# Yukun-Huang/DreamWaltz-G

Hardware: AMD Instinct MI355X
Metric: SDS steps/sec @512^2, 100k Gaussians, SD1.5+ControlNet; raster Mpix/s vs HBM roofline (higher is better)
Workload: dtype f32x

## Files before the change

dreamwaltz-g_amd/csrc/gemm.hip:

```cpp
#include "dwg_common.h"
#include "dwg_prof_internal.h"
#include "../../include/dwg_gemm.h"
#include <cstdlib>
#include <type_traits>

#if defined(DWG_GEMM_X_TU)
#include "dwg_xfmt.h"
typedef _Float16 HT;
#define DWG_DTYPE_HALF DWG_DTYPE_F32X
#define DWG_MFMA16(a, b, c) __builtin_amdgcn_mfma_f32_32x32x16_f16(a, b, c, 0, 0, 0)
#define DWG_HALF_NAME "f32x"
#elif defined(DWG_GEMM_F16_TU)
typedef _Float16 HT;
#define DWG_DTYPE_HALF DWG_DTYPE_F16
#define DWG_MFMA16(a, b, c) __builtin_amdgcn_mfma_f32_32x32x16_f16(a, b, c, 0, 0, 0)
#define DWG_HALF_NAME "f16"
#else
typedef __bf16 HT;
#define DWG_DTYPE_HALF DWG_DTYPE_BF16
#define DWG_MFMA16(a, b, c) __builtin_amdgcn_mfma_f32_32x32x16_bf16(a, b, c, 0, 0, 0)
#define DWG_HALF_NAME "bf16"
#endif

namespace {

typedef __attribute__((ext_vector_type(8))) HT bf16x8;
typedef __attribute__((ext_vector_type(16))) float f32x16;

struct ConvP {
    int enabled, Cin, Hin, Win, Hout, Wout, KH, KW, stride, pad_t, pad_l, dil;
    int up;
    int cin1;
    const void* A2;
};

struct GemmP {
    const void* A; const void* B; void* C; const void* bias; const void* residual;
    int M, N, K;
    long long sam, sak, sbn, sbk, ldc, ldr;
    int nb2;
    long long bA1, bA2, bB1, bB2, bC1, bC2, bR1, bR2;
    int act; float alpha;
    int out_bf16, res_bf16, bias_per_row, splitk, accumulate;
    float* ws;
    int bias_row_div;
    long long bias_ld;
    ConvP conv;
};

__device__ __forceinline__ float bf2f(HT x) { return (float)x; }
__device__ __forceinline__ HT f2bf(float x) { return (HT)x; }

struct bf16x4_t { HT v[4]; };
#ifdef DWG_GEMM_X_TU
__device__ __forceinline__ float ld_half1(const void* base, long long i) { return dwg_x_get1(base, i); }
__device__ __forceinline__ void st_half1(void* base, long long i, float v) { dwg_x_put1(base, i, v); }
__device__ __forceinline__ void ld_half4(const void* base, long long i, float (&v)[4]) { dwg_x_get4(base, i, v); }
__device__ __forceinline__ void st_half4(void* base, long long i, const float (&v)[4]) { dwg_x_put4(base, i, v); }
#else
__device__ __forceinline__ float ld_half1(const void* base, long long i) { return bf2f(reinterpret_cast<const HT*>(base)[i]); }
__device__ __forceinline__ void st_half1(void* base, long long i, float v) { reinterpret_cast<HT*>(base)[i] = f2bf(v); }
__device__ __forceinline__ void ld_half4(const void* base, long long i, float (&v)[4]) {
    const bf16x4_t r = *reinterpret_cast<const bf16x4_t*>(reinterpret_cast<const HT*>(base) + i);
// ... 59 lines not shown

    __device__ __forceinline__ void init(const T* base_, long long srow_, long long sk_, int nrows_, int r0_, int kbeg, int kend_,
                                         const ConvP& cv) {
        base = base_; srow = srow_; sk = sk_; nrows = nrows_; r0 = r0_; kend = kend_;
        const int tid = threadIdx.x;
        if (MODE == MODE_KVEC) {
            kcur = kbeg + (tid % CPR) * VEC;
#pragma unroll
            for (int i = 0; i < NCH; i++) {
                int r = r0 + tid / CPR + i * RPI;
                rowptr[i] = r < nrows ? base + (long long)r * srow : nullptr;
            }
        } else if (MODE == MODE_CONV) {
            kcur = kbeg + (tid % CPR) * VEC;
            const int hw = cv.Hout * cv.Wout;
#pragma unroll
            for (int i = 0; i < NCH; i++) {
                int r = r0 + tid / CPR + i * RPI;
                rok[i] = r < nrows;
                int rr = rok[i] ? r : 0;
                int img = rr / hw, rem = rr - img * hw;
                int oy = rem / cv.Wout, ox = rem - oy * cv.Wout;
                iy0[i] = oy * cv.stride - cv.pad_t; ix0[i] = ox * cv.stride - cv.pad_l;
                pix0[i] = (long long)img * cv.Hin * cv.Win;
            }
            int tap = kcur / cv.Cin;
            ci = kcur - tap * cv.Cin; ky = tap / cv.KW; kx = tap - ky * cv.KW;
        } else {
            kcur = kbeg;
        }
    }

    __device__ __forceinline__ void advance(const ConvP& cv) {
        kcur += BK;
        if (MODE == MODE_CONV) {
            ci += BK;
            while (ci >= cv.Cin) { ci -= cv.Cin; if (++kx == cv.KW) { kx = 0; ++ky; } }
        }
// ... 75 lines not shown
        acc = DWG_MFMA16(a, b, acc);
    }
}
template <>
__device__ __forceinline__ void mma_tile<float>(const float* sa, const float* sb, int lane, f32x16& acc) {
    constexpr int LDT = TT<float>::BK + TT<float>::PAD;
    const float* pa = sa + (lane & 31) * LDT + (lane >> 5);
    const float* pb = sb + (lane & 31) * LDT + (lane >> 5);
#pragma unroll
    for (int ks = 0; ks < TT<float>::BK / 2; ks++)
        acc = __builtin_amdgcn_mfma_f32_32x32x2f32(pa[ks * 2], pb[ks * 2], acc, 0, 0, 0);
}

template <bool LIGHT = false>
__device__ __forceinline__ void epilogue_store(const GemmP& p, float v, int row, int col, long long coff, long long roff) {
    const long long ci = coff + (long long)row * p.ldc + col;
    if (p.bias) v += reinterpret_cast<const float*>(p.bias)[p.bias_row_div > 0 ? (long long)(row / p.bias_row_div) * p.bias_ld + col
                                                                             : (p.bias_per_row ? row : col)];
    v = apply_act<LIGHT>(v, p.act);
    if (p.residual) {
        const long long ri = roff + (long long)row * p.ldr + col;
        v += p.res_bf16 ? ld_half1(p.residual, ri) : reinterpret_cast<const float*>(p.residual)[ri];
    }
    if (p.out_bf16) st_half1(p.C, ci, v);
    else if (p.accumulate) reinterpret_cast<float*>(p.C)[ci] += v;
    else reinterpret_cast<float*>(p.C)[ci] = v;
}

__device__ __forceinline__ bool epilogue_vec_ok(const GemmP& p, long long coff, long long roff) {
    bool ok = (p.N & 3) == 0 && (p.ldc & 3) == 0 && (coff & 3) == 0 && ((uintptr_t)p.C & 15) == 0;
    if (p.residual) ok = ok && (p.ldr & 3) == 0 && (roff & 3) == 0 && ((uintptr_t)p.residual & 15) == 0;
    return ok;
}

template <bool LIGHT = false>
__device__ __forceinline__ void epilogue_store4(const GemmP& p, float (&v)[4], int row, int col, long long coff, long long roff, bool vec_ok) {
    if (!vec_ok || col + 3 >= p.N) {
#pragma unroll
        for (int e = 0; e < 4; e++)
            if (col + e < p.N) epilogue_store<LIGHT>(p, v[e], row, col + e, coff, roff);
        return;
    }
    if (p.bias) {
        const float* b = reinterpret_cast<const float*>(p.bias);
        if (p.bias_row_div > 0) {
// ... 8 lines not shown
    }
#pragma unroll
    for (int e = 0; e < 4; e++) v[e] = apply_act<LIGHT>(v[e], p.act);
    if (p.residual) {
        const long long ri = roff + (long long)row * p.ldr + col;
        if (p.res_bf16) {
            float r[4];
            ld_half4(p.residual, ri, r);
#pragma unroll
            for (int e = 0; e < 4; e++) v[e] += r[e];
        } else {
            float4 r = *reinterpret_cast<const float4*>(reinterpret_cast<const float*>(p.residual) + ri);
            v[0] += r.x; v[1] += r.y; v[2] += r.z; v[3] += r.w;
        }
    }
    const long long ci = coff + (long long)row * p.ldc + col;
    if (p.out_bf16) {
        st_half4(p.C, ci, v);
    } else {
        float4* dst = reinterpret_cast<float4*>(reinterpret_cast<float*>(p.C) + ci);
        float4 o = make_float4(v[0], v[1], v[2], v[3]);
        if (p.accumulate) { float4 c = *dst; o.x += c.x; o.y += c.y; o.z += c.z; o.w += c.w; }
        *dst = o;
    }
}

template <int BN, int BM = 128> struct EpiLds {
    static constexpr int LDC = BN + 4;
    static constexpr int passes(size_t lds_bytes) {
        return lds_bytes >= (size_t)BM * LDC * 4 ? 1 : (lds_bytes >= (size_t)(BM / 2) * LDC * 4 ? 2 : 4);
    }
// ... 29 lines not shown
                    *reinterpret_cast<float4*>(dst + j * 32 + 8 * r4) =
                        make_float4(acc[i][j][4 * r4], acc[i][j][4 * r4 + 1], acc[i][j][4 * r4 + 2], acc[i][j][4 * r4 + 3]);
        }
        __syncthreads();
        if (geglu) {
            constexpr int G = C4 / 2, RSTEP = NT / G;
            const int o4 = tid & (G - 1), rl0 = tid / G;
            const int b = o4 >> 3, w = (o4 & 7) * 4;
            const int colp = n0 + b * 64 + w;
            if (colp + 35 < p.N) {
                float bh[4] = {0.f, 0.f, 0.f, 0.f}, bg[4] = {0.f, 0.f, 0.f, 0.f};
                if (bias) {
#pragma unroll
                    for (int e = 0; e < 4; e++) { bh[e] = bias[colp + e]; bg[e] = bias[colp + 32 + e]; }
                }
                const bool vec_store = ((p.ldc | coff) & 3) == 0 && ((uintptr_t)p.C & 7) == 0;
#pragma unroll 2
                for (int rl = rl0; rl < PR; rl += RSTEP) {
                    const int row = row_of(q * PR + rl);
                    if (row < 0) continue;
                    const float4 h = *reinterpret_cast<const float4*>(sC + rl * LDC + b * 64 + w);
                    const float4 g = *reinterpret_cast<const float4*>(sC + rl * LDC + b * 64 + 32 + w);
                    const float hv[4] = {h.x, h.y, h.z, h.w}, gv[4] = {g.x, g.y, g.z, g.w};
                    float v[4];
#pragma unroll
                    for (int e = 0; e < 4; e++) {
                        const float a = fmaf(hv[e], p.alpha, bh[e]);
                        const float gg = fmaf(gv[e], p.alpha, bg[e]);
                        v[e] = a * 0.5f * gg * (1.f + dwg_erf_fast(gg * 0.70710678118654752f));
                    }
                    const long long ci = coff + (long long)row * p.ldc + (n0 + b * 64) / 2 + w;
                    if (p.out_bf16) {
                        if (vec_store) {
                            st_half4(p.C, ci, v);
                        } else {
#pragma unroll
                            for (int e = 0; e < 4; e++) st_half1(p.C, ci + e, v[e]);
                        }
                    } else {
#pragma unroll
                        for (int e = 0; e < 4; e++) reinterpret_cast<float*>(p.C)[ci + e] = v[e];
                    }
                }
            }
            continue;
        }
// ... 28 lines not shown
#pragma unroll
                        for (int e = 0; e < 4; e++) v[e] = apply_act<LIGHT>(v[e], p.act);
                    }
                    if (p.residual) {
                        const long long ri = roff + (long long)row * p.ldr + col;
                        if (p.res_bf16) {
                            float r[4];
                            ld_half4(p.residual, ri, r);
#pragma unroll
                            for (int e = 0; e < 4; e++) v[e] += r[e];
                        } else {
                            const float4 r = *reinterpret_cast<const float4*>(reinterpret_cast<const float*>(p.residual) + ri);
                            v[0] += r.x; v[1] += r.y; v[2] += r.z; v[3] += r.w;
                        }
                    }
                    const long long ci = coff + (long long)row * p.ldc + col;
                    if (p.out_bf16) {
                        st_half4(p.C, ci, v);
                    } else {
                        *reinterpret_cast<float4*>(reinterpret_cast<float*>(p.C) + ci) = make_float4(v[0], v[1], v[2], v[3]);
                    }
                }
            }
            continue;
        }
#pragma unroll 1
        for (int idx = tid; idx < PR * C4; idx += NT) {
            const int rl = idx / C4, c4 = idx - rl * C4;
            const int row = row_of(q * PR + rl), col = n0 + c4 * 4;
            if (row < 0 || col >= p.N) continue;
            const float4 a = *reinterpret_cast<const float4*>(sC + rl * LDC + c4 * 4);
            float v[4] = {a.x * p.alpha, a.y * p.alpha, a.z * p.alpha, a.w * p.alpha};
            if (p.splitk > 1) {
                if (p.ws) {
                    float* dst = p.ws + ((long long)ks_id * p.M + row) * p.N + col;
                    if ((p.N & 3) == 0) *reinterpret_cast<float4*>(dst) = make_float4(v[0], v[1], v[2], v[3]);
                    else {
#pragma unroll
                        for (int e = 0; e < 4; e++) if (col + e < p.N) dst[e] = v[e];
                    }
                } else {
#pragma unroll
                    for (int e = 0; e < 4; e++)
                        if (col + e < p.N) atomicAdd(reinterpret_cast<float*>(p.C) + coff + (long long)row * p.ldc + col + e, v[e]);
                }
                continue;
            }
            epilogue_store4<LIGHT>(p, v, row, col, coff, roff, vec_ok);
        }
    }
}

__global__ __launch_bounds__(256) void k_splitk_epilogue(GemmP p) {
    const long long n = (long long)p.M * p.N;
    if ((p.N & 3) == 0) {
        const bool vec_ok = epilogue_vec_ok(p, 0, 0);
        const int N4 = p.N >> 2;
        const long long n4 = n >> 2;
        for (long long i = (long long)blockIdx.x * 256 + threadIdx.x; i < n4; i += (long long)gridDim.x * 256) {
// ... 117 lines not shown

    __device__ __forceinline__ void init(const HT* base_, long long srow, int nrows, int r0, int kbeg, int kend_, const ConvP& cv) {
        static_assert(NJ % 2 == 0, "row-block parity must equal j parity");
        base = base_; kend = kend_;
        const int lane = threadIdx.x & 63, wave = threadIdx.x >> 6, sub = lane >> 3;
        const int lg0 = (lane & 7) ^ (sub >> 1);
        kc[0] = kbeg + lg0 * 8; kc[1] = kbeg + (lg0 ^ 4) * 8;
        if (!CONV) {
#pragma unroll
            for (int j = 0; j < NJ; j++) {
                int r = r0 + (wave * NJ + j) * 8 + sub;
                rowptr[j] = r < nrows ? base + (long long)r * srow : nullptr;
            }
        } else {
            const int hw = cv.Hout * cv.Wout;
#pragma unroll
            for (int j = 0; j < NJ; j++) {
                int r = r0 + (wave * NJ + j) * 8 + sub;
                rok[j] = r < nrows;
                int rr = rok[j] ? r : 0;
                int img = rr / hw, rem = rr - img * hw;
                int oy = rem / cv.Wout, ox = rem - oy * cv.Wout;
                iy0[j] = oy * cv.stride - cv.pad_t; ix0[j] = ox * cv.stride - cv.pad_l;
                pix0[j] = (long long)img * cv.Hin * cv.Win;
            }
#pragma unroll
            for (int q = 0; q < 2; q++) {
                int tap = kc[q] / cv.Cin;
                ci[q] = kc[q] - tap * cv.Cin; ky[q] = tap / cv.KW; kx[q] = tap - ky[q] * cv.KW;
            }
        }
    }
    __device__ __forceinline__ void advance(const ConvP& cv) {
        kc[0] += 64; kc[1] += 64;
        if (CONV) {
#pragma unroll
            for (int q = 0; q < 2; q++) {
                ci[q] += 64;
// ... 40 lines not shown
struct GldsConvFast {
    static constexpr int NJ = ROWS / (8 * NW);
    const unsigned char* pb[NJ];
    const unsigned char* pb2[CAT ? NJ : 1];
    unsigned int mask[NJ];
    int kcur, kend, tap, ci, ky, kx;

    __device__ __forceinline__ void init(const HT* base, long long, int nrows, int r0, int kbeg, int kend_, const ConvP& cv) {
        static_assert(NJ % 2 == 0, "row-block parity must equal j parity");
        const int lane = threadIdx.x & 63, wave = threadIdx.x >> 6, sub = lane >> 3;
        const int lg0 = (lane & 7) ^ (sub >> 1);
        kcur = kbeg; kend = kend_;
        tap = kbeg / cv.Cin; ci = kbeg - tap * cv.Cin; ky = tap / cv.KW; kx = tap - ky * cv.KW;
        const int hw = cv.Hout * cv.Wout;
        const int cs1 = CAT ? cv.cin1 : cv.Cin;
#pragma unroll
        for (int j = 0; j < NJ; j++) {
            const int r = r0 + (wave * NJ + j) * 8 + sub;
            const bool rok = r < nrows;
            const int rr = rok ? r : 0;
            const int img = rr / hw, rem = rr - img * hw;
            const int oy = rem / cv.Wout, ox = rem - oy * cv.Wout;
            const int iy0 = oy * cv.stride - cv.pad_t, ix0 = ox * cv.stride - cv.pad_l;
            unsigned int m = 0;
            for (int t = 0, y = 0; y < cv.KH; y++)
                for (int x = 0; x < cv.KW; x++, t++) {
                    const int iy = iy0 + y, ix = ix0 + x;
                    if (rok && iy >= 0 && iy < cv.Hin && ix >= 0 && ix < cv.Win) m |= 1u << t;
                }
            mask[j] = m;
            const long long pix = ((long long)img * cv.Hin + iy0) * cv.Win + ix0;
            pb[j] = reinterpret_cast<const unsigned char*>(base) + (pix * cs1 + (lg0 ^ ((j & 1) << 2)) * 8) * 2;
            if (CAT) pb2[j] = reinterpret_cast<const unsigned char*>(cv.A2) + (pix * (cv.Cin - cv.cin1) + (lg0 ^ ((j & 1) << 2)) * 8) * 2;
        }
    }
    __device__ __forceinline__ void advance(const ConvP& cv) {
        kcur += 64; ci += 64;
        const int w = ci >= cv.Cin ? 1 : 0;
// ... 724 lines not shown
    if (akind == 3) f(std::integral_constant<int, 3>{});
    else if (akind == 2) f(std::integral_constant<int, 2>{});
    else if (akind == 1) f(std::integral_constant<int, 1>{});
    else f(std::integral_constant<int, 0>{});
}

}

#ifdef DWG_GEMM_X_TU
static bool x_physical(const dwg_gemm_desc* d, dwg_gemm_desc* o) {
    if (!d) return false;
    *o = *d;
    if (d->dtype != DWG_DTYPE_F32X) return false;
    if (d->K % 8 || d->a_k_stride != 1 || d->b_k_stride != 1) return false;
    if ((d->a_row_stride | d->b_row_stride | d->a_batch1_stride | d->a_batch2_stride | d->b_batch1_stride | d->b_batch2_stride) % 8) return false;
    if (d->out_dtype == DWG_DTYPE_F32X && ((d->ldc | d->c_batch1_stride | d->c_batch2_stride) % 8 || ((uintptr_t)d->C % 16))) return false;
    if (d->residual && d->residual_dtype == DWG_DTYPE_F32X &&
        (((d->ldr ? d->ldr : d->ldc) | d->r_batch1_stride | d->r_batch2_stride) % 8 || ((uintptr_t)d->residual % 16))) return false;
    if (d->act == DWG_ACT_GEGLU_PAIR && d->out_dtype == DWG_DTYPE_F32X && d->N % 16) return false;
    if (d->conv_enabled && (d->conv_cin % 8 || (d->A2 && d->conv_cin1 % 8))) return false;
    o->K = 2 * d->K;
    o->a_row_stride = 2 * d->a_row_stride; o->b_row_stride = 2 * d->b_row_stride;
    o->a_batch1_stride = 2 * d->a_batch1_stride; o->a_batch2_stride = 2 * d->a_batch2_stride;
    o->b_batch1_stride = 2 * d->b_batch1_stride; o->b_batch2_stride = 2 * d->b_batch2_stride;
    o->conv_cin = 2 * d->conv_cin; o->conv_cin1 = 2 * d->conv_cin1;
    return true;
}
#endif

extern "C" {

// ... 40 lines not shown
    if (d && d->dtype == DWG_DTYPE_F32X) return dwg_gemm_x(d, stream_);
#endif
#ifdef DWG_GEMM_X_TU
    dwg_gemm_desc xd;
    if (!x_physical(d, &xd)) return DWG_E_ARG;
    d = &xd;
#endif
    if (!d || !d->A || !d->B || !d->C) return DWG_E_ARG;
    if (d->M < 0 || d->N < 0 || d->K < 0 || d->batch1 < 1 || d->batch2 < 1 || d->plan_m < 0) return DWG_E_ARG;
    if (d->M == 0 || d->N == 0) return DWG_OK;
    if (d->dtype != DWG_DTYPE_F32 && d->dtype != DWG_DTYPE_HALF) return DWG_E_ARG;
    if (d->splitk > 1 && !d->workspace && (d->out_dtype != DWG_DTYPE_F32 || d->bias || d->residual || d->act)) return DWG_E_ARG;
    if (d->accumulate && d->out_dtype != DWG_DTYPE_F32) return DWG_E_ARG;
    if (d->act == DWG_ACT_GEGLU_PAIR && (d->N % 64 != 0 || d->residual || d->splitk > 1 || d->bias_per_row || d->bias_row_div)) return DWG_E_ARG;
    if ((uintptr_t)d->workspace & 15) return DWG_E_ARG;
    GemmP p;
    p.A = d->A; p.B = d->B; p.C = d->C; p.bias = d->bias; p.residual = d->residual;
    p.M = d->M; p.N = d->N; p.K = d->K;
    p.sam = d->a_row_stride; p.sak = d->a_k_stride; p.sbn = d->b_row_stride; p.sbk = d->b_k_stride;
    p.ldc = d->ldc; p.ldr = d->ldr ? d->ldr : d->ldc;
    p.nb2 = d->batch2;
    p.bA1 = d->a_batch1_stride; p.bA2 = d->a_batch2_stride; p.bB1 = d->b_batch1_stride; p.bB2 = d->b_batch2_stride;
    p.bC1 = d->c_batch1_stride; p.bC2 = d->c_batch2_stride; p.bR1 = d->r_batch1_stride; p.bR2 = d->r_batch2_stride;
    p.act = d->act; p.alpha = d->alpha;
    p.out_bf16 = d->out_dtype == DWG_DTYPE_HALF; p.res_bf16 = d->residual_dtype == DWG_DTYPE_HALF;
    p.bias_per_row = d->bias_per_row; p.accumulate = d->accumulate;
    const bool plain1x1 = d->conv_enabled && d->conv_kh == 1 && d->conv_kw == 1 && d->conv_stride == 1 && d->conv_pad_t == 0 &&
                          d->conv_pad_l == 0 && d->conv_in_dilation <= 1 && d->conv_in_upsample <= 1 && !d->A2 && d->conv_hout == d->conv_hin &&
                          d->conv_wout == d->conv_win && d->K == d->conv_cin && batch_of(d) == 1;
    if (plain1x1) { p.sam = d->conv_cin; p.sak = 1; }
    p.conv.enabled = d->conv_enabled && !plain1x1;
    p.conv.Cin = d->conv_cin; p.conv.Hin = d->conv_hin; p.conv.Win = d->conv_win; p.conv.Hout = d->conv_hout;
    p.conv.Wout = d->conv_wout; p.conv.KH = d->conv_kh; p.conv.KW = d->conv_kw; p.conv.stride = d->conv_stride;
    p.conv.pad_t = d->conv_pad_t; p.conv.pad_l = d->conv_pad_l; p.conv.dil = d->conv_in_dilation > 1 ? d->conv_in_dilation : 1;
    p.conv.up = d->conv_in_upsample > 1 ? d->conv_in_upsample : 1;
    p.conv.A2 = d->A2; p.conv.cin1 = d->A2 ? d->conv_cin1 : d->conv_cin;
    p.bias_row_div = d->bias_row_div; p.bias_ld = d->bias_ld > 0 ? d->bias_ld : d->N;
    Plan pl;
    dwg_gemm_desc pd = *d;
    if (d->plan_m > d->M) pd.M = d->plan_m;
    const int rc = make_plan(&pd, p, pl);
    if (rc != DWG_OK) return rc;
    p.splitk = pl.splitk;
    p.ws = pl.slabs ? reinterpret_cast<float*>(d->workspace) : nullptr;
    const int batch = batch_of(d);
    hipStream_t stream = (hipStream_t)stream_;
    const char* name = d->name ? d->name : (d->conv_enabled ? "conv_igemm" : "gemm");
    switch (pl.fam) {
        case FAM_PATCH2:
            if (pl.nw == 8) launch_conv3x3_patch2<128, 8, 4>(p, stream, name);
            else if (pl.bn == 64) launch_conv3x3_patch2<64, 4, 4>(p, stream, name);
            else launch_conv3x3_patch2<128, 4, 2>(p, stream, name);
// ... 30 lines not shown
```

dreamwaltz-g_amd/gemm.py:

```python
import ctypes

import torch

from . import _lib

F32, BF16, F16, F32X = 0, 1, 2, 3
ACT = {None: 0, "none": 0, "relu": 1, "leaky_relu": 2, "silu": 3, "gelu": 4, "sigmoid": 5, "geglu_pair": 6}


class GemmDesc(ctypes.Structure):
    _fields_ = [
        ("A", ctypes.c_void_p), ("B", ctypes.c_void_p), ("C", ctypes.c_void_p), ("bias", ctypes.c_void_p),
        ("residual", ctypes.c_void_p),
        ("M", ctypes.c_int32), ("N", ctypes.c_int32), ("K", ctypes.c_int32),
        ("a_row_stride", ctypes.c_int64), ("a_k_stride", ctypes.c_int64), ("b_row_stride", ctypes.c_int64),
        ("b_k_stride", ctypes.c_int64), ("ldc", ctypes.c_int64), ("ldr", ctypes.c_int64),
        ("batch1", ctypes.c_int32), ("batch2", ctypes.c_int32),
        ("a_batch1_stride", ctypes.c_int64), ("a_batch2_stride", ctypes.c_int64), ("b_batch1_stride", ctypes.c_int64),
        ("b_batch2_stride", ctypes.c_int64), ("c_batch1_stride", ctypes.c_int64), ("c_batch2_stride", ctypes.c_int64),
        ("r_batch1_stride", ctypes.c_int64), ("r_batch2_stride", ctypes.c_int64),
        ("dtype", ctypes.c_int32), ("out_dtype", ctypes.c_int32), ("residual_dtype", ctypes.c_int32),
        ("act", ctypes.c_int32), ("alpha", ctypes.c_float), ("bias_per_row", ctypes.c_int32),
        ("splitk", ctypes.c_int32), ("accumulate", ctypes.c_int32),
        ("conv_enabled", ctypes.c_int32), ("conv_cin", ctypes.c_int32), ("conv_hin", ctypes.c_int32),
        ("conv_win", ctypes.c_int32), ("conv_hout", ctypes.c_int32), ("conv_wout", ctypes.c_int32),
        ("conv_kh", ctypes.c_int32), ("conv_kw", ctypes.c_int32), ("conv_stride", ctypes.c_int32),
        ("conv_pad_t", ctypes.c_int32), ("conv_pad_l", ctypes.c_int32), ("conv_in_dilation", ctypes.c_int32),
        ("conv_in_upsample", ctypes.c_int32), ("A2", ctypes.c_void_p), ("conv_cin1", ctypes.c_int32),
        ("bias_row_div", ctypes.c_int32), ("bias_ld", ctypes.c_int64),
        ("workspace", ctypes.c_void_p), ("workspace_bytes", ctypes.c_size_t),
        ("name", ctypes.c_char_p), ("plan_m", ctypes.c_int32),
    ]


def _dt(t):
    if t.dtype == torch.float32:
        return F32
    if t.dtype == torch.bfloat16:
        return BF16
    if t.dtype == torch.float16:
        return F16
    if t.dtype == torch.int32:
        return F32X
    raise TypeError("dwg gemm supports float32, bfloat16, float16 and f32x (int32-typed, xfmt.py) tensors, got %s" % t.dtype)


def _stream(t):
    return ctypes.c_void_p(torch.cuda.current_stream(t.device).cuda_stream)


def gemm_raw(A, B, C, M, N, K, a_strides, b_strides, ldc, bias=None, residual=None, ldr=0, act=None, alpha=1.0,
             batch=(1, 1), a_batch=(0, 0), b_batch=(0, 0), c_batch=(0, 0), r_batch=(0, 0), bias_per_row=False, splitk=1,
             accumulate=False, conv=None, name=None, conv_upsample=1, A2=None, cin1=0, bias_row_div=0, bias_ld=0, plan_m=0, run=True):
    if not A.is_cuda:
        raise RuntimeError("dreamwaltz_g_amd GEMM runs on the GPU only (HIP kernels)")
    d = GemmDesc()
    d.A, d.B, d.C = A.data_ptr(), B.data_ptr(), C.data_ptr()
    d.bias = bias.data_ptr() if bias is not None else None
    d.residual = residual.data_ptr() if residual is not None else None
    d.M, d.N, d.K = M, N, K
    d.a_row_stride, d.a_k_stride = a_strides
    d.b_row_stride, d.b_k_stride = b_strides
    d.ldc, d.ldr = ldc, ldr
    d.batch1, d.batch2 = batch
    d.a_batch1_stride, d.a_batch2_stride = a_batch
    d.b_batch1_stride, d.b_batch2_stride = b_batch
    d.c_batch1_stride, d.c_batch2_stride = c_batch
    d.r_batch1_stride, d.r_batch2_stride = r_batch
# ... 5 lines not shown
    d.alpha = alpha
    d.bias_per_row = int(bias_per_row)
    d.splitk = splitk
    d.accumulate = int(accumulate)
    if conv is not None:
        d.conv_enabled = 1
        (d.conv_cin, d.conv_hin, d.conv_win, d.conv_hout, d.conv_wout, d.conv_kh, d.conv_kw, d.conv_stride, d.conv_pad_t,
         d.conv_pad_l, d.conv_in_dilation) = conv
    d.conv_in_upsample = conv_upsample
    if A2 is not None:
        d.A2 = A2.data_ptr(); d.conv_cin1 = cin1
    d.bias_row_div = bias_row_div
    d.bias_ld = bias_ld
    d.name = name.encode() if name else None
    d.plan_m = plan_m
    if not run:
        return d
    _lib.check(_lib.lib().dwg_gemm(ctypes.byref(d), _stream(A)), "dwg_gemm")
    return C


def run_desc(d, stream):
    rc = _lib.lib().dwg_gemm(ctypes.byref(d), stream)
    if rc != 0:
        raise RuntimeError("dwg_gemm failed with DWG error %d" % rc)


def linear(x, w, bias=None, act=None, out_dtype=None, residual=None, out=None, name=None):
    K = x.shape[-1]
    x2 = x.reshape(-1, K)
# ... 25 lines not shown
```

dreamwaltz-g_amd/sd15.py:

```python
import ctypes
import os
import math
from collections import OrderedDict
from dataclasses import dataclass
from typing import Dict, List, Optional, Tuple

import torch

from . import _lib, gemm, xfmt

BF16 = torch.bfloat16

TORCH_DTYPE = {"bf16": torch.bfloat16, "f32": torch.float32, "f16": torch.float16, "f32x": xfmt.DTYPE}
DT_CODE = {"f32": 0, "bf16": 1, "f16": 2, "f32x": 3}


def dtype_name(dtype) -> str:
    names = {"bf16": "bf16", "bfloat16": "bf16", torch.bfloat16: "bf16", "f32": "f32", "fp32": "f32", "float32": "f32", torch.float32: "f32",
             "f16": "f16", "fp16": "f16", "float16": "f16", "half": "f16", torch.float16: "f16", "f32x": "f32x", "fp32x": "f32x"}
    if dtype not in names:
        raise ValueError("plan dtype must be one of bf16 / f32 / f16 / f32x, got %r" % (dtype,))
    return names[dtype]


# ... 417 lines not shown

    def conv_dgrad_s2(self, name, py, px):
        key = ("dgrad_s2", name, py, px)
        if key not in self.cache:
            w = self.sd[name + ".weight"].float()
            kmap = {0: [2, 0], 1: [1]}
            kys, kxs = kmap[py], kmap[px]
            cy, cx = w.shape[0], w.shape[1]
            wp = torch.zeros(_pad8(cx), len(kys), len(kxs), _pad8(cy))
            for ty, ky in enumerate(kys):
                for tx, kx in enumerate(kxs):
                    wp[:cx, ty, tx, :cy] = w[:, :, ky, kx].t()
            self.cache[key] = self._to_dev(wp)
        return self.cache[key]

    def lin(self, *names):
        key = ("lin",) + names
        if key not in self.cache:
            self.cache[key] = self._to_dev(torch.cat([self.sd[n + ".weight"].float().reshape(self.sd[n + ".weight"].shape[0], -1)
                                                      for n in names], 0))
        return self.cache[key]

    def lin_t(self, name):
        key = ("lin_t", name)
        if key not in self.cache:
            w = self.sd[name + ".weight"].float()
            self.cache[key] = self._to_dev(w.reshape(w.shape[0], -1).t().contiguous())
        return self.cache[key]

    def lin_geglu(self, name):
# ... 7 lines not shown
        return self.cache[key]

    def f32(self, name):
        if name not in self.cache:
            self.cache[name] = self.sd[name].float().to(self.device).contiguous()
        return self.cache[name]

    def bias_cat(self, *names):
        key = ("bias",) + names
        if key not in self.cache:
            self.cache[key] = torch.cat([self.sd[n].float() for n in names], 0).to(self.device).contiguous()
        return self.cache[key]


class Builder:
    def __init__(self, plan: Plan, w: Weights, groups=32, prefix="net"):
        self.p, self.w, self.groups, self.prefix = plan, w, groups, prefix
        self.L = _lib.lib()
        self.full_batch = None

    def _plan_rows(self, b, m):
        return m * self.full_batch // b if self.full_batch and b < self.full_batch and self.full_batch % b == 0 else 0

    def _conv_tag(self, tag, KH, Ho, stride, dil, KW=None):
        if tag:
            return tag
        KW = KH if KW is None else KW
        base = "conv3x3" if KH == 3 else ("conv1x1" if KH * KW == 1 else "conv%dx%d" % (KH, KW))
        return "%s%s_%s_r%d" % (base, "s2" if stride == 2 else ("T" if dil > 1 else ""), self.prefix, Ho)

    def conv(self, x, name, stride=1, pad=1, act=None, residual=None, upsample=1, bias_img=None, out_dtype=None, out_hw=None,
             pad_tl=None, r_batch_bcast=False, weight=None, bias=True, in_dilation=1, tag=None):
        B, H, W, C = x.shape
        self.p.scope = name
        wt = self.w.conv(name) if weight is None else weight
        Cout, KH, KW, Cin = wt.shape
        assert Cin == C, (name, Cin, C)
        Hv, Wv = ((H - 1) * in_dilation + 1) * upsample, ((W - 1) * in_dilation + 1) * upsample
        pt, pl = (pad, pad) if pad_tl is None else pad_tl
        if out_hw is None:
            Ho, Wo = (Hv + 2 * pad - KH) // stride + 1, (Wv + 2 * pad - KW) // stride + 1
        else:
            Ho, Wo = out_hw
        y = self.p.buf(B, Ho, Wo, Cout, dtype=out_dtype)
        b = None
        if bias_img is None and bias:
            b = self.w.f32(name + ".bias")
            if b.numel() < Cout:
                b = None
        conv = (C, H, W, Ho, Wo, KH, KW, stride, pt, pl, in_dilation)
        K = KH * KW * C
        if r_batch_bcast and KH * KW == 1 and stride == 1 and pad == 0 and pad_tl is None and upsample == 1 and in_dilation == 1 and out_hw is None:
            Vr = int(residual.shape[0])
            assert B % Vr == 0 and bias_img is None, (B, Vr)
            Mr = Vr * H * W
            d = gemm.gemm_raw(x, wt, y, Mr, Cout, K, (C, 1), (K, 1), Cout, bias=b, residual=residual, ldr=Cout, act=act, batch=(B // Vr, 1),
                              a_batch=(Mr * C, 0), c_batch=(Mr * Cout, 0), r_batch=(0, 0), name=self._conv_tag(tag, KH, Ho, stride, in_dilation, KW),
                              run=False)
        elif r_batch_bcast:
            Vr = int(residual.shape[0])
            assert B % Vr == 0, (B, Vr)
            d = gemm.gemm_raw(x, wt, y, Ho * Wo, Cout, K, (0, 1), (K, 1), Cout, bias=b, residual=residual, ldr=Cout, act=act,
                              batch=(B // Vr, Vr), a_batch=(Vr * H * W * C, H * W * C), c_batch=(Vr * Ho * Wo * Cout, Ho * Wo * Cout),
                              r_batch=(0, Ho * Wo * Cout), conv=conv,
                              conv_upsample=upsample, name=self._conv_tag(tag, KH, Ho, stride, in_dilation, KW), run=False)
        else:
            kw = {}
            if bias_img is not None:
                kw = dict(bias=bias_img[0], bias_row_div=Ho * Wo, bias_ld=bias_img[1])
            else:
                kw = dict(bias=b)
            d = gemm.gemm_raw(x, wt, y, B * Ho * Wo, Cout, K, (0, 1), (K, 1), Cout, residual=residual,
                              ldr=Cout if residual is not None else 0, act=act, conv=conv, conv_upsample=upsample,
                              name=self._conv_tag(tag, KH, Ho, stride, in_dilation, KW), plan_m=self._plan_rows(B, B * Ho * Wo), run=False, **kw)
        self.p.add_gemm(d)
        return y

    def linear(self, x, wt, bias=None, act=None, residual=None, out_dtype=None, tag="linear"):
        K = x.shape[-1]
        M = x.numel() // K
        N = wt.shape[0]
        Nout = N // 2 if act == "geglu_pair" else N
        y = self.p.buf(*x.shape[:-1], Nout, dtype=out_dtype)
        if residual is not None and residual.numel() != M * Nout:
            R = (M * Nout) // residual.numel()
            Mr = M // R
            assert Mr * R == M and residual.numel() == Mr * Nout and x.is_contiguous(), (M, Nout, tuple(residual.shape))
            d = gemm.gemm_raw(x, wt, y, Mr, N, K, (K, 1), (wt.stride(0), 1), Nout, bias=bias, residual=residual, ldr=Nout, act=act, batch=(R, 1),
                              a_batch=(Mr * K, 0), c_batch=(Mr * Nout, 0), r_batch=(0, 0), name=tag, run=False)
# ... 108 lines not shown
            assert a.shape[0] % b.shape[0] == 0 and a.shape[1:-1] == b.shape[1:-1], (tuple(a.shape), tuple(b.shape))
            self.p.add_call(self.L.dwg_concat_channels_bcast, a.numel() // Ca, b.numel() // Cb, Ca * k2, Cb * k2, pp(a), pp(b), pp(y))
            return y
        self.p.add_call(self.L.dwg_concat_channels, a.numel() // Ca, Ca * k2, Cb * k2, pp(a), pp(b), pp(y))
        return y

    def add(self, a, b):
        y = self.p.buf(*a.shape)
        pp = lambda t: ctypes.c_void_p(t.data_ptr())
        self.p.add_call(self.L.dwg_add_dt, self.p.dt, a.numel(), pp(a), pp(b), pp(y))
        return y

    def conv_dgrad_s2(self, dy, name):
        B, Ho, Wo, _ = dy.shape
        subs = []
        for py in (0, 1):
            for px in (0, 1):
                wt = self.w.conv_dgrad_s2(name, py, px)
                subs.append(self.conv(dy, None, weight=wt, bias=False, stride=1, pad_tl=(wt.shape[1] - 1, wt.shape[2] - 1),
                                      out_hw=(Ho, Wo)))
        C = subs[0].shape[-1]
        out = self.p.buf(B, 2 * Ho, 2 * Wo, C)
        pp = lambda t: ctypes.c_void_p(t.data_ptr())
        self.p.add_call(self.L.dwg_interleave2x2, B, Ho, Wo, C * (self.p.esize // 2), pp(subs[0]), pp(subs[1]), pp(subs[2]), pp(subs[3]), pp(out))
        return out

    def transpose(self, x):
        B, R, C = x.shape
        y = self.p.buf(B, C, R)
        pp = lambda t: ctypes.c_void_p(t.data_ptr())
        self.p.add_call(self.L.dwg_transpose_dt, self.p.dt, B, R, C, pp(x), x.stride(1), x.stride(0), pp(y), R, C * R)
        return y

    def cast_bf16(self, x):
        if self.p.dtype_name == "f32":
# ... 105 lines not shown
            if cfg.attn_blocks[i]:
                h = b.transformer(h, "down_blocks.%d.attentions.%d" % (i, j), text, cfg.heads)
            skips.append(h)
        if i != nb - 1:
            h = b.conv(h, "down_blocks.%d.downsamplers.0.conv" % i, stride=2)
            skips.append(h)
    h = b.resnet(h, "mid_block.resnets.0", temb.bias_for("mid_block.resnets.0"))
    h = b.transformer(h, "mid_block.attentions.0", text, cfg.heads)
    h = b.resnet(h, "mid_block.resnets.1", temb.bias_for("mid_block.resnets.1"))
    return skips, h


class DenoiserPlan:

    def __init__(self, cfg: UNetConfig, unet_sd, cn_sd, device, batch=2, latent_hw=64, text_len=77, dtype="bf16", views=1, weights=None,
                 shared_prefix=False):
        self.cfg, self.device, self.B, self.hw, self.views = cfg, device, batch, latent_hw, int(views)
        self.shared_prefix = bool(shared_prefix)
        if self.shared_prefix and batch != 2 * self.views:
            raise ValueError("a shared-prefix plan runs the CFG pair of each view: batch must be 2 * views, got batch %d for %d view(s)" % (batch, self.views))
        if self.shared_prefix and dtype_name(dtype) == "f32":
            raise NotImplementedError("shared_prefix: the exact-f32 plans run attention on dwg_gemm, whose two batch levels are image x head")
        self._temb_table = None
        self.temb_rows = 1001
        assert batch % self.views == 0, (batch, views)
        self.plan = Plan(device, dtype)
        p = self.plan
        self.pre = Plan(device, dtype)
        self._pre_event, self._pre_ready, self._pre_stream = None, False, None
        wu, wc = weights if weights is not None else (Weights(unet_sd, device, dtype), Weights(cn_sd, device, dtype))
        self.weights = (wu, wc)
        bu, bc = Builder(p, wu, cfg.groups, "unet"), Builder(p, wc, cfg.groups, "cnet")
        pu, pc = Builder(self.pre, wu, cfg.groups, "unet"), Builder(self.pre, wc, cfg.groups, "cnet")
        if self.shared_prefix:
            bu.full_batch = bc.full_batch = batch
        B, hw = batch, latent_hw
        self.latents = p.buf(self.views if self.shared_prefix else B, hw, hw, _pad8(cfg.in_channels), zero=True)
        self.text = p.buf(B, text_len, cfg.cross_dim)
        self.cond_scale = 2 ** (len(cfg.cond_channels) - 1)
        self.cond = p.buf(self.views, hw * self.cond_scale, hw * self.cond_scale, _pad8(cfg.cond_in_channels), zero=True)
        self._lat_stage, self._cond_stage = p.stage_like(self.latents), p.stage_like(self.cond)
        up_names = []
        rev_attn = list(reversed(cfg.attn_blocks))
        for i in range(len(cfg.block_out_channels)):
            for j in range(cfg.layers_per_block + 1):
                up_names.append("up_blocks.%d.resnets.%d" % (i, j))
        nb = len(cfg.block_out_channels)
# ... 85 lines not shown
            self._store_prelude_inputs(t, text, cond_nchw)

    def run(self):
        if self._pre_ready:
            if self._pre_event is not None:
                torch.cuda.current_stream(self.device).wait_event(self._pre_event)
        else:
            self.pre.run()
        self._pre_ready, self._pre_event = False, None
        self.plan.run()
        return self.eps.permute(0, 3, 1, 2)


class VAEEncoderPlan:

    def __init__(self, cfg: VAEConfig, sd, device, image_hw=512, dtype="bf16", batch=1, weights=None):
        self.cfg, self.device, self.hw, self.B = cfg, device, image_hw, int(batch)
        self.fwd, self.bwd = Plan(device, dtype), Plan(device, dtype)
        w = weights if weights is not None else Weights(sd, device, dtype)
        self.weights = w
        f, r = Builder(self.fwd, w, cfg.groups, "vaef"), Builder(self.bwd, w, cfg.groups, "vaeb")
        self.x = self.fwd.buf(self.B, image_hw, image_hw, 8, zero=True)
        self._x_stage = self.fwd.stage_like(self.x)
        boc = cfg.block_out_channels
        tape = []

        def conv_f(xin, name, **kw):
            y = f.conv(xin, name, **kw)
            return y

        def resnet_f(xin, pre):
            C = xin.shape[-1]
            n1, s1 = f.groupnorm(xin, pre + ".norm1", 1e-6, True, keep_stats=True)
            h1 = f.conv(n1, pre + ".conv1")
            n2, s2 = f.groupnorm(h1, pre + ".norm2", 1e-6, True, keep_stats=True)
            Cout = h1.shape[-1]
# ... 159 lines not shown
```

include/dwg_gemm.h:

```cpp
#ifndef DWG_GEMM_H
#define DWG_GEMM_H
#include "dwg_types.h"
#ifdef __cplusplus
extern "C" {
#endif


#define DWG_ACT_NONE 0
#define DWG_ACT_RELU 1
#define DWG_ACT_LEAKY_RELU 2
#define DWG_ACT_SILU 3
#define DWG_ACT_GELU 4
#define DWG_ACT_SIGMOID 5
#define DWG_ACT_GEGLU_PAIR 6

typedef struct dwg_gemm_desc {
    const void* A; const void* B; void* C;
    const float* bias;
    const void* residual;
    int32_t M, N, K;
    int64_t a_row_stride, a_k_stride, b_row_stride, b_k_stride, ldc, ldr;
    int32_t batch1, batch2;
    int64_t a_batch1_stride, a_batch2_stride, b_batch1_stride, b_batch2_stride, c_batch1_stride, c_batch2_stride,
        r_batch1_stride, r_batch2_stride;
// ... 4 lines not shown
    float alpha;
    int32_t bias_per_row;
    int32_t splitk;
    int32_t accumulate;
    int32_t conv_enabled, conv_cin, conv_hin, conv_win, conv_hout, conv_wout, conv_kh, conv_kw, conv_stride, conv_pad_t,
        conv_pad_l, conv_in_dilation;
    int32_t conv_in_upsample;
    const void* A2;
    int32_t conv_cin1;
    int32_t bias_row_div;
    int64_t bias_ld;
    void* workspace;
    size_t workspace_bytes;
    const char* name;
    int32_t plan_m;
} dwg_gemm_desc;

int dwg_gemm(const dwg_gemm_desc* desc, dwg_stream_t stream);

size_t dwg_gemm_workspace_bytes(const dwg_gemm_desc* desc);

#ifdef __cplusplus
}
#endif
#endif
```

Baseline: 40.33.

## Fold nearest-upsample into 2x2 phase convolutions and write strided dgrad outputs in place

A 3x3 convolution after 2x nearest upsampling becomes four 2x2 phase convolutions on the low-resolution input. The weights are pre-summed per phase, and each phase's output is scattered into the interleaved high-resolution buffer through a new row-run output stride. This cuts MACs by more than half and removes the upsampled-input addressing. The same run-stride store also lets the stride-2 dgrad sub-convolutions write directly into the interleaved output, dropping the separate gather/interleave pass. Both paths are gated by size, dtype and legacy flags, and the new descriptor fields and kernel branches add some complexity to every GEMM epilogue.

```diff
diff --git a/dreamwaltz-g_amd/csrc/gemm.hip b/dreamwaltz-g_amd/csrc/gemm.hip
--- a/dreamwaltz-g_amd/csrc/gemm.hip
+++ b/dreamwaltz-g_amd/csrc/gemm.hip
@@ -32,7 +32,13 @@
     int up;
     int cin1;
     const void* A2;
+    int phases;
 };
+
+__device__ __forceinline__ void conv_pads(const ConvP& cv, int& pad_t, int& pad_l) {
+    pad_t = cv.pad_t; pad_l = cv.pad_l;
+    if (cv.phases) { pad_t = 1 - (int)(blockIdx.z >> 1); pad_l = 1 - (int)(blockIdx.z & 1); }
+}
 
 struct GemmP {
     const void* A; const void* B; void* C; const void* bias; const void* residual;
@@ -45,8 +51,15 @@
     float* ws;
     int bias_row_div;
     long long bias_ld;
+    int c_run;
+    long long c_run_stride;
     ConvP conv;
 };
+
+__device__ __forceinline__ long long c_row_off(const GemmP& p, int row) {
+    if (p.c_run > 0) { const int run = row / p.c_run; return run * p.c_run_stride + (long long)(row - run * p.c_run) * p.ldc; }
+    return (long long)row * p.ldc;
+}
 
 __device__ __forceinline__ float bf2f(HT x) { return (float)x; }
 __device__ __forceinline__ HT f2bf(float x) { return (HT)x; }
@@ -136,6 +149,8 @@
         } else if (MODE == MODE_CONV) {
             kcur = kbeg + (tid % CPR) * VEC;
             const int hw = cv.Hout * cv.Wout;
+            int pad_t, pad_l;
+            conv_pads(cv, pad_t, pad_l);
 #pragma unroll
             for (int i = 0; i < NCH; i++) {
                 int r = r0 + tid / CPR + i * RPI;
@@ -143,7 +158,7 @@
                 int rr = rok[i] ? r : 0;
                 int img = rr / hw, rem = rr - img * hw;
                 int oy = rem / cv.Wout, ox = rem - oy * cv.Wout;
-                iy0[i] = oy * cv.stride - cv.pad_t; ix0[i] = ox * cv.stride - cv.pad_l;
+                iy0[i] = oy * cv.stride - pad_t; ix0[i] = ox * cv.stride - pad_l;
                 pix0[i] = (long long)img * cv.Hin * cv.Win;
             }
             int tap = kcur / cv.Cin;
@@ -249,7 +264,7 @@
 
 template <bool LIGHT = false>
 __device__ __forceinline__ void epilogue_store(const GemmP& p, float v, int row, int col, long long coff, long long roff) {
-    const long long ci = coff + (long long)row * p.ldc + col;
+    const long long ci = coff + c_row_off(p, row) + col;
     if (p.bias) v += reinterpret_cast<const float*>(p.bias)[p.bias_row_div > 0 ? (long long)(row / p.bias_row_div) * p.bias_ld + col
                                                                              : (p.bias_per_row ? row : col)];
     v = apply_act<LIGHT>(v, p.act);
@@ -263,7 +278,7 @@
 }
 
 __device__ __forceinline__ bool epilogue_vec_ok(const GemmP& p, long long coff, long long roff) {
-    bool ok = (p.N & 3) == 0 && (p.ldc & 3) == 0 && (coff & 3) == 0 && ((uintptr_t)p.C & 15) == 0;
+    bool ok = (p.N & 3) == 0 && ((p.ldc | p.c_run_stride) & 3) == 0 && (coff & 3) == 0 && ((uintptr_t)p.C & 15) == 0;
     if (p.residual) ok = ok && (p.ldr & 3) == 0 && (roff & 3) == 0 && ((uintptr_t)p.residual & 15) == 0;
     return ok;
 }
@@ -302,7 +317,7 @@
             v[0] += r.x; v[1] += r.y; v[2] += r.z; v[3] += r.w;
         }
     }
-    const long long ci = coff + (long long)row * p.ldc + col;
+    const long long ci = coff + c_row_off(p, row) + col;
     if (p.out_bf16) {
         st_half4(p.C, ci, v);
     } else {
@@ -362,7 +377,7 @@
 #pragma unroll
                     for (int e = 0; e < 4; e++) { bh[e] = bias[colp + e]; bg[e] = bias[colp + 32 + e]; }
                 }
-                const bool vec_store = ((p.ldc | coff) & 3) == 0 && ((uintptr_t)p.C & 7) == 0;
+                const bool vec_store = ((p.ldc | p.c_run_stride | coff) & 3) == 0 && ((uintptr_t)p.C & 7) == 0;
 #pragma unroll 2
                 for (int rl = rl0; rl < PR; rl += RSTEP) {
                     const int row = row_of(q * PR + rl);
@@ -377,7 +392,7 @@
                         const float gg = fmaf(gv[e], p.alpha, bg[e]);
                         v[e] = a * 0.5f * gg * (1.f + dwg_erf_fast(gg * 0.70710678118654752f));
                     }
-                    const long long ci = coff + (long long)row * p.ldc + (n0 + b * 64) / 2 + w;
+                    const long long ci = coff + c_row_off(p, row) + (n0 + b * 64) / 2 + w;
                     if (p.out_bf16) {
                         if (vec_store) {
                             st_half4(p.C, ci, v);
@@ -436,7 +451,7 @@
                             v[0] += r.x; v[1] += r.y; v[2] += r.z; v[3] += r.w;
                         }
                     }
-                    const long long ci = coff + (long long)row * p.ldc + col;
+                    const long long ci = coff + c_row_off(p, row) + col;
                     if (p.out_bf16) {
                         st_half4(p.C, ci, v);
                     } else {
@@ -464,7 +479,7 @@
                 } else {
 #pragma unroll
                     for (int e = 0; e < 4; e++)
-                        if (col + e < p.N) atomicAdd(reinterpret_cast<float*>(p.C) + coff + (long long)row * p.ldc + col + e, v[e]);
+                        if (col + e < p.N) atomicAdd(reinterpret_cast<float*>(p.C) + coff + c_row_off(p, row) + col + e, v[e]);
                 }
                 continue;
             }
@@ -612,6 +627,8 @@
             }
         } else {
             const int hw = cv.Hout * cv.Wout;
+            int pad_t, pad_l;
+            conv_pads(cv, pad_t, pad_l);
 #pragma unroll
             for (int j = 0; j < NJ; j++) {
                 int r = r0 + (wave * NJ + j) * 8 + sub;
@@ -619,7 +636,7 @@
                 int rr = rok[j] ? r : 0;
                 int img = rr / hw, rem = rr - img * hw;
                 int oy = rem / cv.Wout, ox = rem - oy * cv.Wout;
-                iy0[j] = oy * cv.stride - cv.pad_t; ix0[j] = ox * cv.stride - cv.pad_l;
+                iy0[j] = oy * cv.stride - pad_t; ix0[j] = ox * cv.stride - pad_l;
                 pix0[j] = (long long)img * cv.Hin * cv.Win;
             }
 #pragma unroll
@@ -690,6 +707,8 @@
         tap = kbeg / cv.Cin; ci = kbeg - tap * cv.Cin; ky = tap / cv.KW; kx = tap - ky * cv.KW;
         const int hw = cv.Hout * cv.Wout;
         const int cs1 = CAT ? cv.cin1 : cv.Cin;
+        int pad_t, pad_l;
+        conv_pads(cv, pad_t, pad_l);
 #pragma unroll
         for (int j = 0; j < NJ; j++) {
             const int r = r0 + (wave * NJ + j) * 8 + sub;
@@ -697,7 +716,7 @@
             const int rr = rok ? r : 0;
             const int img = rr / hw, rem = rr - img * hw;
             const int oy = rem / cv.Wout, ox = rem - oy * cv.Wout;
-            const int iy0 = oy * cv.stride - cv.pad_t, ix0 = ox * cv.stride - cv.pad_l;
+            const int iy0 = oy * cv.stride - pad_t, ix0 = ox * cv.stride - pad_l;
             unsigned int m = 0;
             for (int t = 0, y = 0; y < cv.KH; y++)
                 for (int x = 0; x < cv.KW; x++, t++) {
@@ -1452,7 +1471,7 @@
     if (d->dtype != DWG_DTYPE_F32X) return false;
     if (d->K % 8 || d->a_k_stride != 1 || d->b_k_stride != 1) return false;
     if ((d->a_row_stride | d->b_row_stride | d->a_batch1_stride | d->a_batch2_stride | d->b_batch1_stride | d->b_batch2_stride) % 8) return false;
-    if (d->out_dtype == DWG_DTYPE_F32X && ((d->ldc | d->c_batch1_stride | d->c_batch2_stride) % 8 || ((uintptr_t)d->C % 16))) return false;
+    if (d->out_dtype == DWG_DTYPE_F32X && ((d->ldc | d->c_batch1_stride | d->c_batch2_stride | d->c_run_stride) % 8 || ((uintptr_t)d->C % 16))) return false;
     if (d->residual && d->residual_dtype == DWG_DTYPE_F32X &&
         (((d->ldr ? d->ldr : d->ldc) | d->r_batch1_stride | d->r_batch2_stride) % 8 || ((uintptr_t)d->residual % 16))) return false;
     if (d->act == DWG_ACT_GEGLU_PAIR && d->out_dtype == DWG_DTYPE_F32X && d->N % 16) return false;
@@ -1523,6 +1542,11 @@
     if (d->accumulate && d->out_dtype != DWG_DTYPE_F32) return DWG_E_ARG;
     if (d->act == DWG_ACT_GEGLU_PAIR && (d->N % 64 != 0 || d->residual || d->splitk > 1 || d->bias_per_row || d->bias_row_div)) return DWG_E_ARG;
     if ((uintptr_t)d->workspace & 15) return DWG_E_ARG;
+    if (d->c_run < 0 || (d->c_run > 0 && d->residual)) return DWG_E_ARG;
+    if (d->conv_up2_phases && !(d->conv_enabled && d->batch1 == 2 && d->batch2 == 2 && d->conv_kh == 2 && d->conv_kw == 2 && d->conv_stride == 1 &&
+                                d->conv_in_dilation <= 1 && d->conv_in_upsample <= 1 && !d->A2 && d->conv_hout == d->conv_hin &&
+                                d->conv_wout == d->conv_win))
+        return DWG_E_ARG;
     GemmP p;
     p.A = d->A; p.B = d->B; p.C = d->C; p.bias = d->bias; p.residual = d->residual;
     p.M = d->M; p.N = d->N; p.K = d->K;
@@ -1544,7 +1568,9 @@
     p.conv.pad_t = d->conv_pad_t; p.conv.pad_l = d->conv_pad_l; p.conv.dil = d->conv_in_dilation > 1 ? d->conv_in_dilation : 1;
     p.conv.up = d->conv_in_upsample > 1 ? d->conv_in_upsample : 1;
     p.conv.A2 = d->A2; p.conv.cin1 = d->A2 ? d->conv_cin1 : d->conv_cin;
+    p.conv.phases = d->conv_up2_phases ? 1 : 0;
     p.bias_row_div = d->bias_row_div; p.bias_ld = d->bias_ld > 0 ? d->bias_ld : d->N;
+    p.c_run = d->c_run; p.c_run_stride = d->c_run > 0 ? d->c_run_stride : 0;
     Plan pl;
     dwg_gemm_desc pd = *d;
     if (d->plan_m > d->M) pd.M = d->plan_m;
diff --git a/dreamwaltz-g_amd/gemm.py b/dreamwaltz-g_amd/gemm.py
--- a/dreamwaltz-g_amd/gemm.py
+++ b/dreamwaltz-g_amd/gemm.py
@@ -30,6 +30,7 @@
         ("bias_row_div", ctypes.c_int32), ("bias_ld", ctypes.c_int64),
         ("workspace", ctypes.c_void_p), ("workspace_bytes", ctypes.c_size_t),
         ("name", ctypes.c_char_p), ("plan_m", ctypes.c_int32),
+        ("c_run", ctypes.c_int32), ("c_run_stride", ctypes.c_int64), ("conv_up2_phases", ctypes.c_int32),
     ]
 
 
@@ -51,7 +52,8 @@
 
 def gemm_raw(A, B, C, M, N, K, a_strides, b_strides, ldc, bias=None, residual=None, ldr=0, act=None, alpha=1.0,
              batch=(1, 1), a_batch=(0, 0), b_batch=(0, 0), c_batch=(0, 0), r_batch=(0, 0), bias_per_row=False, splitk=1,
-             accumulate=False, conv=None, name=None, conv_upsample=1, A2=None, cin1=0, bias_row_div=0, bias_ld=0, plan_m=0, run=True):
+             accumulate=False, conv=None, name=None, conv_upsample=1, A2=None, cin1=0, bias_row_div=0, bias_ld=0, plan_m=0, c_run=0,
+             c_run_stride=0, conv_up2_phases=False, run=True):
     if not A.is_cuda:
         raise RuntimeError("dreamwaltz_g_amd GEMM runs on the GPU only (HIP kernels)")
     d = GemmDesc()
@@ -87,6 +89,8 @@
     d.bias_ld = bias_ld
     d.name = name.encode() if name else None
     d.plan_m = plan_m
+    d.c_run, d.c_run_stride = c_run, c_run_stride
+    d.conv_up2_phases = int(conv_up2_phases)
     if not run:
         return d
     _lib.check(_lib.lib().dwg_gemm(ctypes.byref(d), _stream(A)), "dwg_gemm")
diff --git a/dreamwaltz-g_amd/sd15.py b/dreamwaltz-g_amd/sd15.py
--- a/dreamwaltz-g_amd/sd15.py
+++ b/dreamwaltz-g_amd/sd15.py
@@ -455,6 +455,21 @@
             self.cache[key] = self._to_dev(wp)
         return self.cache[key]
 
+    def conv_up2_phases(self, name):
+        key = ("up2_phases", name)
+        if key not in self.cache:
+            w = self.sd[name + ".weight"].double()
+            taps = {0: ([0], [1, 2]), 1: ([0, 1], [2])}
+            cout, cin = w.shape[0], w.shape[1]
+            wp = torch.zeros(2, 2, cout, 2, 2, _pad8(cin), dtype=torch.float64)
+            for a in (0, 1):
+                for b in (0, 1):
+                    for ty, kys in enumerate(taps[a]):
+                        for tx, kxs in enumerate(taps[b]):
+                            wp[a, b, :, ty, tx, :cin] = w[:, :, kys][:, :, :, kxs].sum((2, 3))
+            self.cache[key] = self._to_dev(wp.float().reshape(2, 2, cout, 4 * _pad8(cin)))
+        return self.cache[key]
+
     def lin(self, *names):
         key = ("lin",) + names
         if key not in self.cache:
@@ -492,8 +507,9 @@
 
 
 class Builder:
-    def __init__(self, plan: Plan, w: Weights, groups=32, prefix="net"):
+    def __init__(self, plan: Plan, w: Weights, groups=32, prefix="net", legacy_routes=False):
         self.p, self.w, self.groups, self.prefix = plan, w, groups, prefix
+        self.legacy_routes = bool(legacy_routes)
         self.L = _lib.lib()
         self.full_batch = None
 
@@ -508,9 +524,12 @@
         return "%s%s_%s_r%d" % (base, "s2" if stride == 2 else ("T" if dil > 1 else ""), self.prefix, Ho)
 
     def conv(self, x, name, stride=1, pad=1, act=None, residual=None, upsample=1, bias_img=None, out_dtype=None, out_hw=None,
-             pad_tl=None, r_batch_bcast=False, weight=None, bias=True, in_dilation=1, tag=None):
+             pad_tl=None, r_batch_bcast=False, weight=None, bias=True, in_dilation=1, tag=None, out=None):
         B, H, W, C = x.shape
         self.p.scope = name
+        if upsample == 2 and self._up2_phases(x, stride, pad, act, residual, bias_img, out_dtype, out_hw, pad_tl, r_batch_bcast, weight,
+                                              in_dilation, out):
+            return self.conv_up2(x, name, tag)
         wt = self.w.conv(name) if weight is None else weight
         Cout, KH, KW, Cin = wt.shape
         assert Cin == C, (name, Cin, C)
@@ -520,7 +539,12 @@
             Ho, Wo = (Hv + 2 * pad - KH) // stride + 1, (Wv + 2 * pad - KW) // stride + 1
         else:
             Ho, Wo = out_hw
-        y = self.p.buf(B, Ho, Wo, Cout, dtype=out_dtype)
+        c_map = {}
+        if out is None:
+            y = self.p.buf(B, Ho, Wo, Cout, dtype=out_dtype)
+        else:
+            assert residual is None and tuple(out.shape) == (B, Ho, Wo, Cout) and out.stride() == (4 * Ho * Wo * Cout, 4 * Wo * Cout, 2 * Cout, 1)
+            y, c_map = out, dict(c_run=Wo, c_run_stride=4 * Wo * Cout, ldc=2 * Cout)
         b = None
         if bias_img is None and bias:
             b = self.w.f32(name + ".bias")
@@ -548,9 +572,33 @@
                 kw = dict(bias=bias_img[0], bias_row_div=Ho * Wo, bias_ld=bias_img[1])
             else:
                 kw = dict(bias=b)
-            d = gemm.gemm_raw(x, wt, y, B * Ho * Wo, Cout, K, (0, 1), (K, 1), Cout, residual=residual,
+            d = gemm.gemm_raw(x, wt, y, B * Ho * Wo, Cout, K, (0, 1), (K, 1), c_map.get("ldc", Cout), residual=residual,
                               ldr=Cout if residual is not None else 0, act=act, conv=conv, conv_upsample=upsample,
-                              name=self._conv_tag(tag, KH, Ho, stride, in_dilation, KW), plan_m=self._plan_rows(B, B * Ho * Wo), run=False, **kw)
+                              name=self._conv_tag(tag, KH, Ho, stride, in_dilation, KW), plan_m=self._plan_rows(B, B * Ho * Wo),
+                              c_run=c_map.get("c_run", 0), c_run_stride=c_map.get("c_run_stride", 0), run=False, **kw)
+        assert not c_map or d.c_run, "in-place phases: the plain convolution call only"
+        self.p.add_gemm(d)
+        return y
+
+    UP2_PHASES_MIN_M = 2048
+
+    def _up2_phases(self, x, stride, pad, act, residual, bias_img, out_dtype, out_hw, pad_tl, r_batch_bcast, weight, in_dilation, out):
+        plain = (stride == 1 and pad == 1 and residual is None and bias_img is None and out_dtype is None and out_hw is None and pad_tl is None
+                 and not r_batch_bcast and weight is None and in_dilation == 1 and out is None)
+        B, H, W, C = x.shape
+        return (plain and not self.legacy_routes and self.p.dtype_name != "f32" and not self._plan_rows(B, 1) and
+                (C * self.p.esize // 2) % 64 == 0 and B * 4 * H * W >= self.UP2_PHASES_MIN_M)
+
+    def conv_up2(self, x, name, tag=None, act=None):
+        B, H, W, C = x.shape
+        self.p.scope = name
+        wt = self.w.conv_up2_phases(name)
+        N, K = wt.shape[2], wt.shape[3]
+        assert K == 4 * C, (name, K, C)
+        y = self.p.buf(B, 2 * H, 2 * W, N)
+        d = gemm.gemm_raw(x, wt, y, B * H * W, N, K, (0, 1), (K, 1), 2 * N, bias=self.w.f32(name + ".bias"), act=act, batch=(2, 2),
+                          a_batch=(0, 0), b_batch=(2 * N * K, N * K), c_batch=(2 * W * N, N), conv=(C, H, W, H, W, 2, 2, 1, 1, 1, 1),
+                          c_run=W, c_run_stride=4 * W * N, conv_up2_phases=True, name=tag or "conv_up2_%s_r%d" % (self.prefix, 2 * H), run=False)
         self.p.add_gemm(d)
         return y
 
@@ -689,11 +737,16 @@
     def conv_dgrad_s2(self, dy, name):
         B, Ho, Wo, _ = dy.shape
         subs = []
+        if not self.legacy_routes:
+            C = self.w.conv_dgrad_s2(name, 0, 0).shape[0]
+            out = self.p.buf(B, 2 * Ho, 2 * Wo, C)
         for py in (0, 1):
             for px in (0, 1):
                 wt = self.w.conv_dgrad_s2(name, py, px)
                 subs.append(self.conv(dy, None, weight=wt, bias=False, stride=1, pad_tl=(wt.shape[1] - 1, wt.shape[2] - 1),
-                                      out_hw=(Ho, Wo)))
+                                      out_hw=(Ho, Wo), out=None if self.legacy_routes else out[:, py::2, px::2]))
+        if not self.legacy_routes:
+            return out
         C = subs[0].shape[-1]
         out = self.p.buf(B, 2 * Ho, 2 * Wo, C)
         pp = lambda t: ctypes.c_void_p(t.data_ptr())
@@ -829,7 +882,7 @@
 class DenoiserPlan:
 
     def __init__(self, cfg: UNetConfig, unet_sd, cn_sd, device, batch=2, latent_hw=64, text_len=77, dtype="bf16", views=1, weights=None,
-                 shared_prefix=False):
+                 shared_prefix=False, legacy_routes=False):
         self.cfg, self.device, self.B, self.hw, self.views = cfg, device, batch, latent_hw, int(views)
         self.shared_prefix = bool(shared_prefix)
         if self.shared_prefix and batch != 2 * self.views:
@@ -845,7 +898,7 @@
         self._pre_event, self._pre_ready, self._pre_stream = None, False, None
         wu, wc = weights if weights is not None else (Weights(unet_sd, device, dtype), Weights(cn_sd, device, dtype))
         self.weights = (wu, wc)
-        bu, bc = Builder(p, wu, cfg.groups, "unet"), Builder(p, wc, cfg.groups, "cnet")
+        bu, bc = Builder(p, wu, cfg.groups, "unet", legacy_routes), Builder(p, wc, cfg.groups, "cnet", legacy_routes)
         pu, pc = Builder(self.pre, wu, cfg.groups, "unet"), Builder(self.pre, wc, cfg.groups, "cnet")
         if self.shared_prefix:
             bu.full_batch = bc.full_batch = batch
@@ -961,12 +1014,12 @@
 
 class VAEEncoderPlan:
 
-    def __init__(self, cfg: VAEConfig, sd, device, image_hw=512, dtype="bf16", batch=1, weights=None):
+    def __init__(self, cfg: VAEConfig, sd, device, image_hw=512, dtype="bf16", batch=1, weights=None, legacy_routes=False):
         self.cfg, self.device, self.hw, self.B = cfg, device, image_hw, int(batch)
         self.fwd, self.bwd = Plan(device, dtype), Plan(device, dtype)
         w = weights if weights is not None else Weights(sd, device, dtype)
         self.weights = w
-        f, r = Builder(self.fwd, w, cfg.groups, "vaef"), Builder(self.bwd, w, cfg.groups, "vaeb")
+        f, r = Builder(self.fwd, w, cfg.groups, "vaef"), Builder(self.bwd, w, cfg.groups, "vaeb", legacy_routes)
         self.x = self.fwd.buf(self.B, image_hw, image_hw, 8, zero=True)
         self._x_stage = self.fwd.stage_like(self.x)
         boc = cfg.block_out_channels
diff --git a/include/dwg_gemm.h b/include/dwg_gemm.h
--- a/include/dwg_gemm.h
+++ b/include/dwg_gemm.h
@@ -42,6 +42,9 @@
     size_t workspace_bytes;
     const char* name;
     int32_t plan_m;
+    int32_t c_run;
+    int64_t c_run_stride;
+    int32_t conv_up2_phases;
 } dwg_gemm_desc;
 
 int dwg_gemm(const dwg_gemm_desc* desc, dwg_stream_t stream);
```

Result: no change. 40.72 (median of 6 runs) (+1.0%).
